# jesusdpa1/ssqueeze_rs

Measured on AMD Instinct MI355X. Metric: TF-bins/sec (ssq_stft, n_fft=1024), higher is better.
Workload: dtype f32

## Files before the change

### ssqueeze_rs_amd/csrc/stft_fused.hip

```cpp
#include "stft_fused_kernel.h"

namespace ssq {

struct Hi1024 {
  static constexpr int N = 1024, L = 64, NF = 513, W = 16, F = 16, PITCH = F + 1, THREADS = W * 64;
  static constexpr int PLANE = NF * PITCH;
  static constexpr int TILE_BYTES = (((2 * PLANE + F) * 4 + 15) / 16) * 16;
  static constexpr int EXH_ELEMS = 64 * 9;
  static constexpr int EXH_BYTES = W * EXH_ELEMS * 8;
  static constexpr int TAB_BYTES = N * 8;
  static constexpr int LDS_BYTES = TILE_BYTES + EXH_BYTES + 2 * TAB_BYTES;
  static constexpr int FRAC = 30, EMIN = -90;
  static_assert(LDS_BYTES <= 160 * 1024, "LDS budget");
};

__device__ __forceinline__ void rows_transpose4(float& r0, float& r1, float& r2, float& r3) {
  auto a = __builtin_amdgcn_permlane32_swap(__float_as_uint(r0), __float_as_uint(r2), false, false);
  auto b = __builtin_amdgcn_permlane32_swap(__float_as_uint(r1), __float_as_uint(r3), false, false);
  auto c = __builtin_amdgcn_permlane16_swap(a[0], b[0], false, false);
  auto d = __builtin_amdgcn_permlane16_swap(a[1], b[1], false, false);
  r0 = __uint_as_float(c[0]);
  r1 = __uint_as_float(c[1]);
  r2 = __uint_as_float(d[0]);
  r3 = __uint_as_float(d[1]);
}

template <bool EDGE, bool LEB, bool WKDBG = false>
__global__ __launch_bounds__(1024, 1) void stft_tx1024_kernel(StftDev<float> p) {
  using H = Hi1024;
  constexpr int THREADS = H::THREADS;
  using T = float;
  constexpr int N = H::N, L = H::L, NF = H::NF, F = H::F, PITCH = H::PITCH;
  __shared__ __attribute__((aligned(16))) unsigned char smem[H::LDS_BYTES];
  int* tile_re = reinterpret_cast<int*>(smem);
  float* col_scale = reinterpret_cast<float*>(tile_re + 2 * H::PLANE);
  cpx<T>* exch_all = reinterpret_cast<cpx<T>*>(smem + H::TILE_BYTES);
  cpx<T>* win_lds = reinterpret_cast<cpx<T>*>(smem + H::TILE_BYTES + H::EXH_BYTES);
  cpx<T>* tw1 = win_lds + N;
  cpx<T>* tw2 = tw1 + 256;

  const int tid = threadIdx.x;
  const int t = tid & 63;
  const int fl = __builtin_amdgcn_readfirstlane(tid >> 6);
  cpx<T>* exch = exch_all + fl * H::EXH_ELEMS;

  for (int i = tid; i < N; i += THREADS) win_lds[i] = p.win2[i];
  if (tid < 256) tw1[tid] = p.tw[((tid & 15) * (tid >> 4) * 4) & (N - 1)];
  for (int i = tid; i < 768; i += THREADS) tw2[i] = p.tw[((i & 255) * ((i >> 8) + 1)) & (N - 1)];
  constexpr long long CELL0 = WKDBG ? 0LL : 0x80000000LL;
  for (int i = tid; i < H::PLANE; i += THREADS) reinterpret_cast<long long*>(tile_re)[i] = CELL0;
  __syncthreads();
  const unsigned bid = blockIdx.x;
  if ((long long)bid >= p.total_tiles) return;

  const long long n_sig = p.total_tiles / p.tiles_per_signal;
  long long sig = (long long)(bid / (unsigned)p.tiles_per_signal);
  int jt = (int)(bid % (unsigned)p.tiles_per_signal);
  auto tile_frame0 = [&](int j) { return ((j < p.ta_n) ? p.ta0 + j : p.tb0 + (j - p.ta_n)) * F; };
  auto load_frame = [&](long long sg, int frame0, T (&xv)[16]) {
    const int frame = frame0 + fl;
    const T* xs = sig_base(p, sg);
    const long long pos0 = (long long)frame * p.hop - p.pad_left + t;
    if constexpr (!EDGE) {
#pragma unroll
      for (int q = 0; q < 16; ++q) xv[q] = xs[pos0 + L * q];
    } else {
      const bool valid = frame < p.n_frames;
      const long long first = pos0 - t;
      if (__all(valid && first >= 0 && first + N <= p.n_signal)) {
#pragma unroll
        for (int q = 0; q < 16; ++q) xv[q] = xs[pos0 + L * q];
      } else {
#pragma unroll
        for (int q = 0; q < 16; ++q) xv[q] = load_padded_flat<false>(xs, pos0 + L * q, p.n_signal, p.padtype, valid);
      }
    }
  };
  T xn[16];
  load_frame(sig, tile_frame0(jt), xn);
  const cpx<T> twr_unused[3][16] = {};

  auto read_out = [&](long long rsig, int rframe0) {
    if constexpr (!EDGE && !WKDBG) {
      if ((p.n_frames & 1) == 0) {
        constexpr int RS2 = THREADS / (F / 2);
        const int fp = tid % (F / 2);
        const int k0 = tid / (F / 2);
        float4* __restrict__ og4 = reinterpret_cast<float4*>(p.out + rsig * (long long)NF * p.n_frames + rframe0 + 2 * fp +
                                                             (long long)k0 * p.n_frames);
        const long long gstep4 = (long long)RS2 * p.n_frames / 2;
        const T sc0 = col_scale[2 * fp], sc1 = col_scale[2 * fp + 1];
        long long* tc = reinterpret_cast<long long*>(tile_re) + k0 * PITCH + 2 * fp;
        auto sweep2 = [&](int j) {
          const long long c0 = tc[j * RS2 * PITCH], c1 = tc[j * RS2 * PITCH + 1];
          tc[j * RS2 * PITCH] = CELL0;
          tc[j * RS2 * PITCH + 1] = CELL0;
          const int r0 = (int)c0 ^ (int)0x80000000, r1 = (int)c1 ^ (int)0x80000000;
          const int i0 = (int)(c0 >> 32), i1 = (int)(c1 >> 32);
          const float4 val = make_float4((T)r0 * sc0, (T)i0 * sc0, (T)r1 * sc1, (T)i1 * sc1);
          typedef float vf4 __attribute__((ext_vector_type(4)));
          const vf4 nv = {val.x, val.y, val.z, val.w};
          __builtin_nontemporal_store(nv, reinterpret_cast<vf4*>(&og4[j * gstep4]));
        };
        constexpr int NFULL2 = NF / RS2;
#pragma unroll
        for (int j = 0; j < NFULL2; ++j) sweep2(j);
        if (k0 + NFULL2 * RS2 < NF) sweep2(NFULL2);
        return;
      }
    }
    constexpr int RSTEP = THREADS / F;
    const int f = tid % F;
    const int k0 = tid / F;
    cpx<T>* __restrict__ og = p.out + rsig * (long long)NF * p.n_frames + rframe0 + f + (long long)k0 * p.n_frames;
    const long long gstep = (long long)RSTEP * p.n_frames;
    const bool fvalid = EDGE ? (rframe0 + f < p.n_frames) : true;
    const T sc = col_scale[f];
    constexpr int NFULL = NF / RSTEP;
    long long* tc = reinterpret_cast<long long*>(tile_re) + k0 * PITCH + f;
    auto sweep = [&](int j) {
      const long long c = tc[j * RSTEP * PITCH];
      tc[j * RSTEP * PITCH] = CELL0;
      if constexpr (WKDBG) {
        if (fvalid) og[j * gstep] = cpx<T>{__int_as_float((int)c), __int_as_float((int)(c >> 32))};
        return;
      }
      const int ire = (int)c ^ (int)0x80000000;
      const int iim = (int)(c >> 32);
      if (fvalid) og[j * gstep] = cpx<T>{(T)ire * sc, (T)iim * sc};
    };
#pragma unroll
    for (int j = 0; j < NFULL; ++j) sweep(j);
    if (k0 + NFULL * RSTEP < NF) sweep(NFULL);
  };

  const int grid_n = (int)gridDim.x;
#pragma unroll 1
  while (true) {
    const int frame0 = tile_frame0(jt);
    const bool valid = EDGE ? (frame0 + fl < p.n_frames) : true;
    long long nsig = sig;
    int njt = jt + grid_n;
    while (njt >= p.tiles_per_signal) {
      njt -= p.tiles_per_signal;
      ++nsig;
    }
    const bool has_next = nsig < n_sig;
    cpx<T> v[16];
#pragma unroll
    for (int q = 0; q < 16; ++q) {
      const cpx<T> wq = win_lds[t + L * q];
      v[q] = {xn[q] * wq.x, xn[q] * wq.y};
    }

    fft_compute<T, 10, 0, false, false>(v, twr_unused, tw1, t);
    {
      cpx<T> nv[16];
      const int rbase = 9 * (t >> 4) + (t & 7);
#pragma unroll
      for (int ph = 0; ph < 2; ++ph) {
#pragma unroll
        for (int u = 0; u < 8; ++u) exch[9 * t + u] = v[8 * ph + u];
        frame_sync<false>();
        if (((t >> 3) & 1) == ph) {
#pragma unroll
          for (int q = 0; q < 16; ++q) nv[q] = exch[rbase + 36 * q];
        }
        frame_sync<false>();
      }
#pragma unroll
      for (int q = 0; q < 16; ++q) v[q] = nv[q];
    }
    if (has_next) load_frame(nsig, tile_frame0(njt), xn);
    fft_compute<T, 10, 1, false, false, true>(v, twr_unused, tw1, t);
    {
#pragma unroll
      for (int uh = 0; uh < 4; ++uh) {
        rows_transpose4(v[4 * uh + 0].x, v[4 * uh + 1].x, v[4 * uh + 2].x, v[4 * uh + 3].x);
        rows_transpose4(v[4 * uh + 0].y, v[4 * uh + 1].y, v[4 * uh + 2].y, v[4 * uh + 3].y);
      }
#define SSQ_SWAP(i, j)       \
  {                          \
    const cpx<T> t_ = v[i];  \
    v[i] = v[j];             \
    v[j] = t_;               \
  }
      SSQ_SWAP(1, 4) SSQ_SWAP(2, 8) SSQ_SWAP(3, 12) SSQ_SWAP(6, 9) SSQ_SWAP(7, 13) SSQ_SWAP(11, 14)
#undef SSQ_SWAP
    }
    fft_compute<T, 10, 2, false, false, true>(v, twr_unused, tw2 - 256, t);

    cpx<T> zp[9];
    {
      const int src = (L - t) & (L - 1);
      zp[8] = v[8];
      if (t == 0) {
#pragma unroll
        for (int j = 8; j < 15; ++j) v[j] = v[j + 1];
        v[15] = v[0];
      }
#pragma unroll
      for (int q = 0; q < 8; ++q) {
        zp[q].x = __shfl(v[15 - q].x, src);
        zp[q].y = __shfl(v[15 - q].y, src);
      }
      v[8] = zp[8];
    }

    {
      cpx<T> cv[9];
      int dstb[9];
      T wdbg[9];
      int kdbg[9];
      T l1 = 0.0f;
      constexpr int CELL = 8;
      const float lane_on = valid ? 1.0f : 0.0f;
      const float sfs0 = (float)t * p.sfs_step, sfs_q = (float)L * p.sfs_step;
      const int neg_last = -(p.n_freqs - 1);
#pragma unroll
      for (int q = 0; q < 9; ++q) {
        const cpx<T> zk = v[q], zn = zp[q];
        const cpx<T> S = {zk.x + zn.x, zk.y - zn.y};
        const cpx<T> dS = {zk.y + zn.y, zn.x - zk.x};
        const float den = S.x * S.x + S.y * S.y;
        const float num = dS.y * S.x - dS.x * S.y;
        const float pd = num * __builtin_amdgcn_rcpf(den * p.two_pi_eff);
        const float d = (sfs0 + (float)q * sfs_q) - pd;
        const float w = fabsf(d);
        float m = fma_clamp01(den, p.keep_big, p.keep_bias) * fma_clamp01(d, 0.0f, 1.0f);
        if constexpr (LEB) m = leb_keep_f32(m, den, w, p.gamma2);
        if (EDGE) m *= lane_on;
        if (q == 8) m *= (t == 0) ? 1.0f : 0.0f;
        const cpx<T> c = LEB ? cpx<T>{p.leb_unit * m, 0.0f} : cpx<T>{S.x * m, S.y * m};
        cv[q] = c;
        int kneg = cvt_floor_i32(__builtin_fmaf(-w, p.inv_dw, 0.5f));
        kneg = kneg < neg_last ? neg_last : kneg;
        if constexpr (LEB) kneg = (w != w) ? 0 : kneg;
        dstb[q] = __mul24(kneg, -(PITCH * CELL)) + fl * CELL;
        l1 += fabsf(c.x) + fabsf(c.y);
        if constexpr (WKDBG) {
          wdbg[q] = w;
          kdbg[q] = (m != 0.0f) ? -kneg : -1;
        }
      }
      const T tot = frame_allreduce<T, L, false>(l1, t, nullptr, t) * p.dw;
      T scale, inv_scale;
      column_scale<T, H::FRAC, H::EMIN>(tot, p.dw, scale, inv_scale);
      if (t == 0 && valid) col_scale[fl] = inv_scale;
      char* ptile = reinterpret_cast<char*>(tile_re);
      if constexpr (WKDBG) {
#pragma unroll
        for (int q = 0; q < 9; ++q) {
          if ((q < 8 || t == 0) && valid) {
            const unsigned lo = (unsigned)__float_as_int(wdbg[q]), hi = (unsigned)__float_as_int((float)kdbg[q]);
            reinterpret_cast<unsigned long long*>(ptile)[(t + L * q) * PITCH + fl] = ((unsigned long long)hi << 32) | lo;
          }
        }
      } else {
#pragma unroll
        for (int q = 0; q < 9; ++q) {
          const int ia = cvt_round_i32(cv[q].x * scale);
          const int ib = LEB ? 0 : cvt_round_i32(cv[q].y * scale);
          if (q < 8 || t == 0) {
            if (LEB) {
              atomicAdd(reinterpret_cast<unsigned*>(ptile + dstb[q]), (unsigned)ia);
            } else {
              const unsigned hi = (unsigned)(ib + (ia >> 31));
              atomicAdd(reinterpret_cast<unsigned long long*>(ptile + dstb[q]),
                        ((unsigned long long)hi << 32) | (unsigned)ia);
            }
          }
        }
      }
    }
    __syncthreads();
    read_out(sig, frame0);
    __syncthreads();
    if (!has_next) break;
    sig = nsig;
    jt = njt;
  }
}

template <typename T>
bool fused_supported(int n_fft) {
  return n_fft >= 64 && n_fft <= 4096 && (n_fft & (n_fft - 1)) == 0;
}

template <typename T, int LOGN>
static FusedLaunchShape shape_one(const StftDev<T>& p0, int cu_count, long long batch) {
  using C = FusedCfg<T, LOGN>;
  FusedLaunchShape s;
  int per_cu = (160 * 1024) / C::LDS_BYTES;
  if (per_cu < 1) per_cu = 1;
  if (per_cu * C::W > 32) per_cu = 32 / C::W;
  bool tx1024 = false;
  if constexpr (sizeof(T) == 4 && LOGN == 10) tx1024 = (p0.out_kind == 0 || p0.out_kind == 3) && p0.n_eff == C::N;
  s.tx1024 = tx1024;
  const int TF = tx1024 ? Hi1024::F : C::F;
  s.tile_frames = TF;
  const long long span = (long long)TF * p0.hop;
  const int tps_all = (p0.n_frames + TF - 1) / TF;
  long long lo = (p0.pad_left + span - 1) / span;
  long long hi_num = p0.n_signal - C::N - (long long)(TF - 1) * p0.hop + p0.pad_left;
  long long hi = hi_num >= 0 ? hi_num / span + 1 : 0;
  const long long full = p0.n_frames / TF;
  if (hi > full) hi = full;
  if (lo > tps_all) lo = tps_all;
  if (hi < lo) hi = lo;
  const long long blocks_one_wave = (long long)cu_count * (tx1024 ? 1 : per_cu);
  bool single_launch = (long long)tps_all * batch <= 4 * blocks_one_wave;
  if (const char* e = std::getenv("SSQ_SINGLE_LAUNCH")) single_launch = std::atoi(e) != 0;
  for (int edge = single_launch ? 1 : 0; edge < 2; ++edge) {
    FusedLaunchShape::Launch l;
    l.edge = edge;
    if (single_launch) {
      l.ta0 = 0;
      l.ta_n = tps_all;
      l.tb0 = 0;
      l.tiles_per_signal = tps_all;
    } else if (!edge) {
      l.ta0 = (int)lo;
      l.ta_n = (int)(hi - lo);
      l.tb0 = 0;
      l.tiles_per_signal = l.ta_n;
    } else {
      l.ta0 = 0;
      l.ta_n = (int)lo;
      l.tb0 = (int)hi;
      l.tiles_per_signal = (int)lo + (tps_all - (int)hi);
    }
    l.total_tiles = (long long)l.tiles_per_signal * batch;
    if (l.total_tiles <= 0) continue;
    l.blocks = tx1024 ? (long long)cu_count : (long long)cu_count * per_cu;
    if (l.blocks > l.total_tiles) l.blocks = l.total_tiles;
    s.launch[s.n_launch++] = l;
  }
  return s;
}

template <typename T, int LOGN>
static hipError_t launch_one(const StftDev<T>& p0, int cu_count, long long batch, hipStream_t stream) {
  using C = FusedCfg<T, LOGN>;
  const FusedLaunchShape s = shape_one<T, LOGN>(p0, cu_count, batch);
  const bool tx1024 = s.tx1024;
  for (int i = 0; i < s.n_launch; ++i) {
    const FusedLaunchShape::Launch& l = s.launch[i];
    const int edge = l.edge;
    StftDev<T> p = p0;
    p.ta0 = l.ta0;
    p.ta_n = l.ta_n;
    p.tb0 = l.tb0;
    p.tiles_per_signal = l.tiles_per_signal;
    p.total_tiles = l.total_tiles;
    const dim3 g((unsigned)l.blocks), b(C::W * 64);
    if constexpr (sizeof(T) == 4 && LOGN == 10) {
      if (tx1024) {
        const dim3 gh((unsigned)l.blocks), bh(Hi1024::THREADS);
        if (p.out_kind == 3) {
          if (edge) hipLaunchKernelGGL((stft_tx1024_kernel<true, false, true>), gh, bh, 0, stream, p);
          else hipLaunchKernelGGL((stft_tx1024_kernel<false, false, true>), gh, bh, 0, stream, p);
        } else if (p.squeezing == 1) {
          if (edge) hipLaunchKernelGGL((stft_tx1024_kernel<true, true>), gh, bh, 0, stream, p);
          else hipLaunchKernelGGL((stft_tx1024_kernel<false, true>), gh, bh, 0, stream, p);
        } else {
          if (edge) hipLaunchKernelGGL((stft_tx1024_kernel<true, false>), gh, bh, 0, stream, p);
          else hipLaunchKernelGGL((stft_tx1024_kernel<false, false>), gh, bh, 0, stream, p);
        }
        const hipError_t eh = hipGetLastError();
        if (eh != hipSuccess) return eh;
        continue;
      }
    }
    if (p.out_kind == 0 && p.squeezing == 1) {
      if (edge) hipLaunchKernelGGL((stft_fused_kernel<T, LOGN, true, true, true>), g, b, 0, stream, p);
      else hipLaunchKernelGGL((stft_fused_kernel<T, LOGN, true, false, true>), g, b, 0, stream, p);
    } else if (p.out_kind == 0) {
      if (edge) hipLaunchKernelGGL((stft_fused_kernel<T, LOGN, true, true, false>), g, b, 0, stream, p);
      else hipLaunchKernelGGL((stft_fused_kernel<T, LOGN, true, false, false>), g, b, 0, stream, p);
    } else if (p.out_kind == 3) {
      if (edge) hipLaunchKernelGGL((stft_fused_kernel<T, LOGN, true, true, false, true>), g, b, 0, stream, p);
      else hipLaunchKernelGGL((stft_fused_kernel<T, LOGN, true, false, false, true>), g, b, 0, stream, p);
    } else {
      if (edge) hipLaunchKernelGGL((stft_fused_kernel<T, LOGN, false, true, false>), g, b, 0, stream, p);
      else hipLaunchKernelGGL((stft_fused_kernel<T, LOGN, false, false, false>), g, b, 0, stream, p);
    }
    const hipError_t e = hipGetLastError();
    if (e != hipSuccess) return e;
  }
  return hipSuccess;
}

template <typename T>
int fused_tile_frames(int n_fft) {
  return for_fused_len(n_fft, 0, [](auto L) { return (int)FusedCfg<T, decltype(L)::value>::F; });
}

template <typename T>
hipError_t launch_stft_fused(const StftDev<T>& p, int n_fft, int cu_count, long long batch, hipStream_t stream) {
  if (p.n_eff != n_fft) return launch_stft_anylen<T>(p, n_fft, cu_count, batch, stream);
  return for_fused_len(n_fft, hipErrorInvalidValue,
                       [&](auto L) { return launch_one<T, decltype(L)::value>(p, cu_count, batch, stream); });
}

template <typename T>
hipError_t fused_launch_shape(const StftDev<T>& p, int n_fft, int cu_count, long long batch, FusedLaunchShape& shape) {
  if (p.n_eff != n_fft) return anylen_launch_shape<T>(p, n_fft, cu_count, batch, shape);
  return for_fused_len(n_fft, hipErrorInvalidValue, [&](auto L) {
    shape = shape_one<T, decltype(L)::value>(p, cu_count, batch);
    return hipSuccess;
  });
}

template bool fused_supported<float>(int);
template bool fused_supported<double>(int);
template int fused_tile_frames<float>(int);
template int fused_tile_frames<double>(int);
template hipError_t launch_stft_fused<float>(const StftDev<float>&, int, int, long long, hipStream_t);
template hipError_t launch_stft_fused<double>(const StftDev<double>&, int, int, long long, hipStream_t);
template hipError_t fused_launch_shape<float>(const StftDev<float>&, int, int, long long, FusedLaunchShape&);
template hipError_t fused_launch_shape<double>(const StftDev<double>&, int, int, long long, FusedLaunchShape&);

}
```

Before: 296.1 billion.

## Use buffer stores for Tx read-out and hoist first FFT pass across tiles

Interior read-out now writes through raw buffer stores with a 32-bit offset descriptor instead of 64-bit pointer arithmetic. The out-of-range tail row is dropped by pointing it at an offset past the buffer limit rather than using a branch. The paired (even n_frames) path becomes a compile-time template choice, selected on the host. The window multiply, first FFT pass and LDS exchange for the next tile are moved to the end of the loop, after read-out, so they can overlap with outstanding stores. This adds kernel variants and a host-side size check that falls back to the edge path for very large outputs.

```diff
diff --git a/ssqueeze_rs_amd/csrc/stft_fused.hip b/ssqueeze_rs_amd/csrc/stft_fused.hip
--- a/ssqueeze_rs_amd/csrc/stft_fused.hip
+++ b/ssqueeze_rs_amd/csrc/stft_fused.hip
@@ -12,6 +12,7 @@
   static constexpr int LDS_BYTES = TILE_BYTES + EXH_BYTES + 2 * TAB_BYTES;
   static constexpr int FRAC = 30, EMIN = -90;
   static_assert(LDS_BYTES <= 160 * 1024, "LDS budget");
+  static bool buffer_readout_ok(int n_frames) { return ((long long)(NF - 1) * n_frames + F) * 8 <= 0x7ffffff0LL; }
 };
 
 __device__ __forceinline__ void rows_transpose4(float& r0, float& r1, float& r2, float& r3) {
@@ -25,8 +26,9 @@
   r3 = __uint_as_float(d[1]);
 }
 
-template <bool EDGE, bool LEB, bool WKDBG = false>
+template <bool EDGE, bool LEB, bool WKDBG = false, bool PAIRED = false>
 __global__ __launch_bounds__(1024, 1) void stft_tx1024_kernel(StftDev<float> p) {
+  static_assert(!PAIRED || (!EDGE && !WKDBG), "the paired read-out is an interior Tx read-out");
   using H = Hi1024;
   constexpr int THREADS = H::THREADS;
   using T = float;
@@ -80,59 +82,132 @@
   load_frame(sig, tile_frame0(jt), xn);
   const cpx<T> twr_unused[3][16] = {};
 
+  constexpr unsigned RO_DROP = 0x7ffffff0u;
+  constexpr int RO_NT = 2;
+  typedef unsigned ro_u4 __attribute__((ext_vector_type(4)));
+  typedef unsigned ro_u2 __attribute__((ext_vector_type(2)));
   auto read_out = [&](long long rsig, int rframe0) {
-    if constexpr (!EDGE && !WKDBG) {
-      if ((p.n_frames & 1) == 0) {
+    if constexpr (!EDGE) {
+      const unsigned row_bytes = (unsigned)p.n_frames * 8u;
+      const auto rsrc = __builtin_amdgcn_make_buffer_rsrc(p.out + rsig * (long long)NF * p.n_frames + rframe0, 0,
+                                                          (NF - 1) * row_bytes + F * 8u, 0x00020000);
+      if constexpr (PAIRED) {
         constexpr int RS2 = THREADS / (F / 2);
+        constexpr int NFULL2 = NF / RS2;
         const int fp = tid % (F / 2);
         const int k0 = tid / (F / 2);
-        float4* __restrict__ og4 = reinterpret_cast<float4*>(p.out + rsig * (long long)NF * p.n_frames + rframe0 + 2 * fp +
-                                                             (long long)k0 * p.n_frames);
-        const long long gstep4 = (long long)RS2 * p.n_frames / 2;
+        const unsigned voff = (unsigned)k0 * row_bytes + 16u * (unsigned)fp;
         const T sc0 = col_scale[2 * fp], sc1 = col_scale[2 * fp + 1];
         long long* tc = reinterpret_cast<long long*>(tile_re) + k0 * PITCH + 2 * fp;
-        auto sweep2 = [&](int j) {
-          const long long c0 = tc[j * RS2 * PITCH], c1 = tc[j * RS2 * PITCH + 1];
+        auto cells2 = [&](int j, long long& c0, long long& c1) {
+          c0 = tc[j * RS2 * PITCH];
+          c1 = tc[j * RS2 * PITCH + 1];
           tc[j * RS2 * PITCH] = CELL0;
           tc[j * RS2 * PITCH + 1] = CELL0;
+        };
+        auto store2 = [&](int j, unsigned vo, long long c0, long long c1) {
           const int r0 = (int)c0 ^ (int)0x80000000, r1 = (int)c1 ^ (int)0x80000000;
           const int i0 = (int)(c0 >> 32), i1 = (int)(c1 >> 32);
-          const float4 val = make_float4((T)r0 * sc0, (T)i0 * sc0, (T)r1 * sc1, (T)i1 * sc1);
-          typedef float vf4 __attribute__((ext_vector_type(4)));
-          const vf4 nv = {val.x, val.y, val.z, val.w};
-          __builtin_nontemporal_store(nv, reinterpret_cast<vf4*>(&og4[j * gstep4]));
+          const ro_u4 val = {__float_as_uint((T)r0 * sc0), __float_as_uint((T)i0 * sc0), __float_as_uint((T)r1 * sc1),
+                             __float_as_uint((T)i1 * sc1)};
+          __builtin_amdgcn_raw_buffer_store_b128(val, rsrc, vo, (unsigned)(j * RS2) * row_bytes, RO_NT);
         };
-        constexpr int NFULL2 = NF / RS2;
-#pragma unroll
-        for (int j = 0; j < NFULL2; ++j) sweep2(j);
-        if (k0 + NFULL2 * RS2 < NF) sweep2(NFULL2);
-        return;
-      }
-    }
-    constexpr int RSTEP = THREADS / F;
-    const int f = tid % F;
-    const int k0 = tid / F;
-    cpx<T>* __restrict__ og = p.out + rsig * (long long)NF * p.n_frames + rframe0 + f + (long long)k0 * p.n_frames;
-    const long long gstep = (long long)RSTEP * p.n_frames;
-    const bool fvalid = EDGE ? (rframe0 + f < p.n_frames) : true;
-    const T sc = col_scale[f];
-    constexpr int NFULL = NF / RSTEP;
-    long long* tc = reinterpret_cast<long long*>(tile_re) + k0 * PITCH + f;
-    auto sweep = [&](int j) {
-      const long long c = tc[j * RSTEP * PITCH];
-      tc[j * RSTEP * PITCH] = CELL0;
-      if constexpr (WKDBG) {
-        if (fvalid) og[j * gstep] = cpx<T>{__int_as_float((int)c), __int_as_float((int)(c >> 32))};
-        return;
-      }
-      const int ire = (int)c ^ (int)0x80000000;
-      const int iim = (int)(c >> 32);
-      if (fvalid) og[j * gstep] = cpx<T>{(T)ire * sc, (T)iim * sc};
-    };
-#pragma unroll
-    for (int j = 0; j < NFULL; ++j) sweep(j);
-    if (k0 + NFULL * RSTEP < NF) sweep(NFULL);
+#pragma unroll
+        for (int j = 0; j < NFULL2; ++j) {
+          long long c0, c1;
+          cells2(j, c0, c1);
+          store2(j, voff, c0, c1);
+        }
+        const bool own = k0 + NFULL2 * RS2 < NF;
+        long long c0 = CELL0, c1 = CELL0;
+        if (own) cells2(NFULL2, c0, c1);
+        store2(NFULL2, own ? voff : RO_DROP, c0, c1);
+      } else {
+        constexpr int RSTEP = THREADS / F;
+        constexpr int NFULL = NF / RSTEP;
+        const int f = tid % F;
+        const int k0 = tid / F;
+        const unsigned voff = (unsigned)k0 * row_bytes + 8u * (unsigned)f;
+        const T sc = col_scale[f];
+        long long* tc = reinterpret_cast<long long*>(tile_re) + k0 * PITCH + f;
+        auto cell = [&](int j) {
+          const long long c = tc[j * RSTEP * PITCH];
+          tc[j * RSTEP * PITCH] = CELL0;
+          return c;
+        };
+        auto store1 = [&](int j, unsigned vo, long long c) {
+          ro_u2 val;
+          if constexpr (WKDBG) {
+            val = ro_u2{(unsigned)c, (unsigned)(c >> 32)};
+          } else {
+            const int ire = (int)c ^ (int)0x80000000;
+            const int iim = (int)(c >> 32);
+            val = ro_u2{__float_as_uint((T)ire * sc), __float_as_uint((T)iim * sc)};
+          }
+          __builtin_amdgcn_raw_buffer_store_b64(val, rsrc, vo, (unsigned)(j * RSTEP) * row_bytes, 0);
+        };
+#pragma unroll
+        for (int j = 0; j < NFULL; ++j) store1(j, voff, cell(j));
+        const bool own = k0 + NFULL * RSTEP < NF;
+        long long c = CELL0;
+        if (own) c = cell(NFULL);
+        store1(NFULL, own ? voff : RO_DROP, c);
+      }
+    } else {
+      constexpr int RSTEP = THREADS / F;
+      const int f = tid % F;
+      const int k0 = tid / F;
+      cpx<T>* __restrict__ og = p.out + rsig * (long long)NF * p.n_frames + rframe0 + f + (long long)k0 * p.n_frames;
+      const long long gstep = (long long)RSTEP * p.n_frames;
+      const bool fvalid = rframe0 + f < p.n_frames;
+      const T sc = col_scale[f];
+      constexpr int NFULL = NF / RSTEP;
+      long long* tc = reinterpret_cast<long long*>(tile_re) + k0 * PITCH + f;
+      auto sweep = [&](int j) {
+        const long long c = tc[j * RSTEP * PITCH];
+        tc[j * RSTEP * PITCH] = CELL0;
+        if constexpr (WKDBG) {
+          if (fvalid) og[j * gstep] = cpx<T>{__int_as_float((int)c), __int_as_float((int)(c >> 32))};
+          return;
+        }
+        const int ire = (int)c ^ (int)0x80000000;
+        const int iim = (int)(c >> 32);
+        if (fvalid) og[j * gstep] = cpx<T>{(T)ire * sc, (T)iim * sc};
+      };
+#pragma unroll
+      for (int j = 0; j < NFULL; ++j) sweep(j);
+      if (k0 + NFULL * RSTEP < NF) sweep(NFULL);
+    }
   };
+
+  cpx<T> v[16];
+  auto front = [&]() {
+#pragma unroll
+    for (int q = 0; q < 16; ++q) {
+      const cpx<T> wq = win_lds[t + L * q];
+      v[q] = {xn[q] * wq.x, xn[q] * wq.y};
+    }
+
+    fft_compute<T, 10, 0, false, false>(v, twr_unused, tw1, t);
+    {
+      cpx<T> nv[16];
+      const int rbase = 9 * (t >> 4) + (t & 7);
+#pragma unroll
+      for (int ph = 0; ph < 2; ++ph) {
+#pragma unroll
+        for (int u = 0; u < 8; ++u) exch[9 * t + u] = v[8 * ph + u];
+        frame_sync<false>();
+        if (((t >> 3) & 1) == ph) {
+#pragma unroll
+          for (int q = 0; q < 16; ++q) nv[q] = exch[rbase + 36 * q];
+        }
+        frame_sync<false>();
+      }
+#pragma unroll
+      for (int q = 0; q < 16; ++q) v[q] = nv[q];
+    }
+  };
+  front();
 
   const int grid_n = (int)gridDim.x;
 #pragma unroll 1
@@ -146,31 +221,6 @@
       ++nsig;
     }
     const bool has_next = nsig < n_sig;
-    cpx<T> v[16];
-#pragma unroll
-    for (int q = 0; q < 16; ++q) {
-      const cpx<T> wq = win_lds[t + L * q];
-      v[q] = {xn[q] * wq.x, xn[q] * wq.y};
-    }
-
-    fft_compute<T, 10, 0, false, false>(v, twr_unused, tw1, t);
-    {
-      cpx<T> nv[16];
-      const int rbase = 9 * (t >> 4) + (t & 7);
-#pragma unroll
-      for (int ph = 0; ph < 2; ++ph) {
-#pragma unroll
-        for (int u = 0; u < 8; ++u) exch[9 * t + u] = v[8 * ph + u];
-        frame_sync<false>();
-        if (((t >> 3) & 1) == ph) {
-#pragma unroll
-          for (int q = 0; q < 16; ++q) nv[q] = exch[rbase + 36 * q];
-        }
-        frame_sync<false>();
-      }
-#pragma unroll
-      for (int q = 0; q < 16; ++q) v[q] = nv[q];
-    }
     if (has_next) load_frame(nsig, tile_frame0(njt), xn);
     fft_compute<T, 10, 1, false, false, true>(v, twr_unused, tw1, t);
     {
@@ -279,6 +329,7 @@
     if (!has_next) break;
     sig = nsig;
     jt = njt;
+    front();
   }
 }
 
@@ -357,15 +408,19 @@
     if constexpr (sizeof(T) == 4 && LOGN == 10) {
       if (tx1024) {
         const dim3 gh((unsigned)l.blocks), bh(Hi1024::THREADS);
+        const bool edge_k = edge || !Hi1024::buffer_readout_ok(p.n_frames);
+        const bool paired = (p.n_frames & 1) == 0;
         if (p.out_kind == 3) {
-          if (edge) hipLaunchKernelGGL((stft_tx1024_kernel<true, false, true>), gh, bh, 0, stream, p);
+          if (edge_k) hipLaunchKernelGGL((stft_tx1024_kernel<true, false, true>), gh, bh, 0, stream, p);
           else hipLaunchKernelGGL((stft_tx1024_kernel<false, false, true>), gh, bh, 0, stream, p);
         } else if (p.squeezing == 1) {
-          if (edge) hipLaunchKernelGGL((stft_tx1024_kernel<true, true>), gh, bh, 0, stream, p);
-          else hipLaunchKernelGGL((stft_tx1024_kernel<false, true>), gh, bh, 0, stream, p);
+          if (edge_k) hipLaunchKernelGGL((stft_tx1024_kernel<true, true>), gh, bh, 0, stream, p);
+          else if (paired) hipLaunchKernelGGL((stft_tx1024_kernel<false, true, false, true>), gh, bh, 0, stream, p);
+          else hipLaunchKernelGGL((stft_tx1024_kernel<false, true, false, false>), gh, bh, 0, stream, p);
         } else {
-          if (edge) hipLaunchKernelGGL((stft_tx1024_kernel<true, false>), gh, bh, 0, stream, p);
-          else hipLaunchKernelGGL((stft_tx1024_kernel<false, false>), gh, bh, 0, stream, p);
+          if (edge_k) hipLaunchKernelGGL((stft_tx1024_kernel<true, false>), gh, bh, 0, stream, p);
+          else if (paired) hipLaunchKernelGGL((stft_tx1024_kernel<false, false, false, true>), gh, bh, 0, stream, p);
+          else hipLaunchKernelGGL((stft_tx1024_kernel<false, false, false, false>), gh, bh, 0, stream, p);
         }
         const hipError_t eh = hipGetLastError();
         if (eh != hipSuccess) return eh;
```

Result: no change. 296.2 billion, median of 2 (+0.0%).
